# MaxChen228/pingpong-selfplay-ai

Measured on AMD Instinct MI355X. Metric: env-steps/sec (whole node) at 65536 arenas, 1/2/4/8 GPUs; CPU-ref baseline, higher is better.
Workload: dtype f64 env state / f32 QNet; 1 GPU; configs[2]: 65536 arenas/GPU, full DQN train_iterative loop (act both players + env tick + PER push/sample + double-DQN update + Adam + target sync); arenas_per_gpu=65536, global_arenas=65536, pool=8, batch=256, updates_per_vector_step=1, memory_size=1000000, parallelism=dp1 (arena shards, 1 all-reduce/update)

## Files before the change

pingpong-selfplay-ai_amd/csrc/pm_mfma.h:

```cpp
#pragma once
#include "pm_dev.h"

namespace pm {

typedef float f32x16 __attribute__((ext_vector_type(16)));
typedef __attribute__((address_space(3))) void lds_void;

constexpr int PLAIN = 4936;
enum : int {
    F_W1 = 0,
    F_W2 = 512,
    F_B1 = 4608,
    F_B2 = 4672,
    F_H = 4736,
    F_BH = 4992,
    F_SIZE = 5008,
};
static_assert(PLAIN + F_SIZE == PM_QNET_NW, "effective weight block size");

__device__ __forceinline__ int rho(int r) { return (r & 3) + 8 * (r >> 2); }

__device__ __forceinline__ float relu(float x) { return __int_as_float(max(__float_as_int(x), 0)); }

__device__ __forceinline__ void write_feature_frag_image(const float* __restrict__ p, float* __restrict__ f) {
    const int t = threadIdx.x, nt = blockDim.x;
    for (int k = t; k < 512; k += nt) {
        const int jt = k >> 8, lane = (k >> 2) & 63, s = k & 3;
        const int row = 32 * jt + (lane & 31), kk = 2 * s + (lane >> 5);
        f[F_W1 + k] = kk == 0 ? p[B1 + row] : p[W1 + row * 7 + kk - 1];
    }
    for (int k = t; k < 4096; k += nt) {
        const int e = k & 3, lane = (k >> 2) & 63, rq = (k >> 8) & 3, tt = (k >> 10) & 1, jt = k >> 11;
        const int row = 32 * jt + (lane & 31), col = 32 * tt + rho(4 * rq + e) + 4 * (lane >> 5);
        f[F_W2 + k] = p[W2 + row * 64 + col];
    }
    for (int k = t; k < 64; k += nt) {
        const int r = k & 15, h = (k >> 4) & 1, jt = k >> 5;
        f[F_B1 + k] = p[B1 + 32 * jt + rho(r) + 4 * h];
        f[F_B2 + k] = p[B2 + 32 * jt + rho(r) + 4 * h];
    }
}
__device__ __forceinline__ void write_feature_frags(const float* __restrict__ p, float* __restrict__ w) {
    for (int k = threadIdx.x; k < PM_QNET_HEAD_OFF; k += blockDim.x) w[k] = p[k];
    write_feature_frag_image(p, w + PLAIN);
}

__device__ __forceinline__ void write_head_frags(const float* heads, float* __restrict__ w) {
    const int t = threadIdx.x, nt = blockDim.x;
    for (int k = t; k < 260; k += nt) w[WH + k] = heads[k];
    float* f = w + PLAIN;
    for (int k = t; k < 256; k += nt) {
        const int c = k & 3, r = (k >> 2) & 15, tt = (k >> 6) & 1, h = k >> 7;
        f[F_H + k] = heads[c * 64 + 32 * tt + rho(r) + 4 * h];
    }
    if (t < 16) f[F_BH + t] = t < 4 ? heads[256 + t] : 0.f;
}

constexpr int kLwChunks = (F_SIZE / 4 + 63) / 64;
constexpr int kLwFloats = kLwChunks * 256;

template <int N>
__device__ __forceinline__ void copy_lds_f32(const float* __restrict__ src, float* dst) {
    const int wv = threadIdx.x >> 6, lane = threadIdx.x & 63, nw = blockDim.x >> 6;
    for (int c = wv; c * 64 < N; c += nw) {
        const int k = min(c * 64 + lane, N - 1);
        __builtin_amdgcn_global_load_lds((const void*)(src + k), (lds_void*)(dst + c * 64), 4, 0, 0);
    }
}
constexpr int pad64(int n) { return (n + 63) / 64 * 64; }
template <int N>
__device__ __forceinline__ void copy_lds_f32x4(const float* __restrict__ src, float* dst) {
    static_assert(N % 4 == 0, "whole float4s");
    const int wv = threadIdx.x >> 6, lane = threadIdx.x & 63, nw = blockDim.x >> 6;
    const float4* s4 = reinterpret_cast<const float4*>(src);
    for (int c = wv; c * 256 < N; c += nw) {
        const int k = min(c * 64 + lane, N / 4 - 1);
        __builtin_amdgcn_global_load_lds((const void*)(s4 + k), (lds_void*)(dst + c * 256), 16, 0, 0);
    }
}
constexpr int pad256(int n) { return (n + 255) / 256 * 256; }

__device__ __forceinline__ void stage_frags_lds(const float* __restrict__ w, float* lw, int rot) {
    const int wv = threadIdx.x >> 6, lane = threadIdx.x & 63, nw = blockDim.x >> 6;
    const float4* src = reinterpret_cast<const float4*>(w + PLAIN);
    float4* lw4 = reinterpret_cast<float4*>(lw);
    rot %= kLwChunks;
    for (int c0 = wv; c0 < kLwChunks; c0 += nw) {
        const int c = c0 + rot < kLwChunks ? c0 + rot : c0 + rot - kLwChunks;
// ... 140 lines not shown
__device__ __forceinline__ void tile_heads(const float* hf, const f32x16 (&c2)[2], int lane, float (&q)[3]) {
    const int h = lane >> 5;
    float v = 0.f, a0 = 0.f, a1 = 0.f, a2 = 0.f;
    const float4* hw = reinterpret_cast<const float4*>(hf + h * 128);
#pragma unroll
    for (int t = 0; t < 2; ++t) {
#pragma unroll
        for (int r = 0; r < 16; ++r) {
            const float x = relu(c2[t][r]);
            const float4 w = hw[t * 16 + r];
            v = fmaf(w.x, x, v);
            a0 = fmaf(w.y, x, a0);
            a1 = fmaf(w.z, x, a1);
            a2 = fmaf(w.w, x, a2);
        }
        __builtin_amdgcn_sched_barrier(0);
    }
    v += __shfl_xor(v, 32);
    a0 += __shfl_xor(a0, 32);
    a1 += __shfl_xor(a1, 32);
    a2 += __shfl_xor(a2, 32);
    v += hf[256];
    a0 += hf[257];
    a1 += hf[258];
    a2 += hf[259];
    const float mean = ((a0 + a1) + a2) / 3.0f;
    q[0] = v + (a0 - mean);
    q[1] = v + (a1 - mean);
    q[2] = v + (a2 - mean);
}

__device__ __forceinline__ void hidden_half(const float* lw, const float (&xs)[4], int lane, int jt, f32x16& c2) {
    const int h = lane >> 5;
    f32x16 c1[2];
    const f32x16 zero = {};
#pragma unroll
    for (int t = 0; t < 2; ++t) {
        const float4 w = reinterpret_cast<const float4*>(lw + F_W1)[t * 64 + lane];
        c1[t] = __builtin_amdgcn_mfma_f32_32x32x2f32(w.x, xs[0], zero, 0, 0, 0);
        c1[t] = __builtin_amdgcn_mfma_f32_32x32x2f32(w.y, xs[1], c1[t], 0, 0, 0);
        c1[t] = __builtin_amdgcn_mfma_f32_32x32x2f32(w.z, xs[2], c1[t], 0, 0, 0);
        c1[t] = __builtin_amdgcn_mfma_f32_32x32x2f32(w.w, xs[3], c1[t], 0, 0, 0);
    }
#pragma unroll
    for (int t = 0; t < 2; ++t)
#pragma unroll
        for (int r = 0; r < 16; ++r) c1[t][r] = relu(c1[t][r]);
    {
        const float4* b = reinterpret_cast<const float4*>(lw + F_B2 + (jt * 2 + h) * 16);
#pragma unroll
        for (int q4 = 0; q4 < 4; ++q4) {
            const float4 v = b[q4];
            c2[4 * q4 + 0] = v.x; c2[4 * q4 + 1] = v.y; c2[4 * q4 + 2] = v.z; c2[4 * q4 + 3] = v.w;
        }
    }
    const float4* w2 = reinterpret_cast<const float4*>(lw + F_W2) + lane + jt * 8 * 64;
    float4 wcur = w2[0];
#pragma unroll
    for (int g = 0; g < 8; ++g) {
        const int t = g >> 2, rq = g & 3;
        const float4 wnext = w2[((g + 1) & 7) * 64];
        c2 = __builtin_amdgcn_mfma_f32_32x32x2f32(wcur.x, c1[t][4 * rq + 0], c2, 0, 0, 0);
        c2 = __builtin_amdgcn_mfma_f32_32x32x2f32(wcur.y, c1[t][4 * rq + 1], c2, 0, 0, 0);
        c2 = __builtin_amdgcn_mfma_f32_32x32x2f32(wcur.z, c1[t][4 * rq + 2], c2, 0, 0, 0);
        c2 = __builtin_amdgcn_mfma_f32_32x32x2f32(wcur.w, c1[t][4 * rq + 3], c2, 0, 0, 0);
        wcur = wnext;
        __builtin_amdgcn_sched_barrier(0);
    }
}

__device__ __forceinline__ void heads_half(const float* hf, const f32x16& c2, int lane, int t, float (&acc)[4]) {
    const float4* hw = reinterpret_cast<const float4*>(hf + (lane >> 5) * 128) + t * 16;
#pragma unroll
    for (int r = 0; r < 16; ++r) {
        const float x = relu(c2[r]);
        const float4 w = hw[r];
        acc[0] = fmaf(w.x, x, acc[0]);
        acc[1] = fmaf(w.y, x, acc[1]);
        acc[2] = fmaf(w.z, x, acc[2]);
        acc[3] = fmaf(w.w, x, acc[3]);
    }
}

__device__ __forceinline__ void heads_finish(const float (&acc)[4], const float* hf, float (&q)[3]) {
    float v = acc[0], a0 = acc[1], a1 = acc[2], a2 = acc[3];
    v += __shfl_xor(v, 32);
    a0 += __shfl_xor(a0, 32);
    a1 += __shfl_xor(a1, 32);
    a2 += __shfl_xor(a2, 32);
    v += hf[256];
    a0 += hf[257];
    a1 += hf[258];
    a2 += hf[259];
    const float mean = ((a0 + a1) + a2) / 3.0f;
    q[0] = v + (a0 - mean);
    q[1] = v + (a1 - mean);
    q[2] = v + (a2 - mean);
}

__device__ __forceinline__ int l2_pos(int u) {
    const int t = u >> 5, v = u & 31, b = (v >> 2) & 1, r = (v & 3) + 4 * (v >> 3);
    return 2 * (16 * t + r) + b;
}
__device__ __forceinline__ int l2_unit(int q) {
    const int i = q >> 1, b = q & 1;
    return 32 * (i >> 4) + rho(i & 15) + 4 * b;
}
__device__ __forceinline__ int head_pos(int u) {
    const int t = u >> 5, v = u & 31;
    return 16 * t + (v & 3) + 4 * (v >> 3);
}

typedef float f32x4v16 __attribute__((ext_vector_type(4)));

template <int NSET>
__device__ __forceinline__ void heads_to_opw(float (&opw)[NSET][2][4][32], int set, const float* hf) {
    const int lane = threadIdx.x & 63;
#pragma unroll
    for (int it = 0; it < 4; ++it) {
        const int idx = it * 64 + lane, h = idx >> 7, j = (idx >> 5) & 3, q = idx & 31;
        opw[set][h][j][q] = hf[(h * 32 + q) * 4 + j];
    }
}

__device__ __forceinline__ float xor16_sum(float v) {
    const auto r = __builtin_amdgcn_permlane16_swap(__float_as_uint(v), __float_as_uint(v), false, false);
    return __uint_as_float(r[0]) + __uint_as_float(r[1]);
}

__device__ __forceinline__ void tile_inputs(const float* __restrict__ o, int h, float (&xs)[4]) {
    xs[0] = h ? o[0] : 1.0f;
    xs[1] = o[1 + h];
    xs[2] = o[3 + h];
    xs[3] = o[5 + h];
}

struct TilePre {
    bool have;
    float xs[4];
};

__device__ __forceinline__ void run_tiles(const float* lw, const float* __restrict__ obs, const int* list, int count,
                                          const TileOut& out, const TilePre pre) {
    const int lane = threadIdx.x & 63, wave = threadIdx.x >> 6, nw = blockDim.x >> 6;
    const int h = lane >> 5, col = lane & 31;
    const int ntiles = (count + 31) >> 5;
    int tl = wave;
    if (tl >= ntiles) return;
    int arena = list[min(tl * 32 + col, count - 1)];
    float xs[4];
    if (pre.have) {
#pragma unroll
        for (int k = 0; k < 4; ++k) xs[k] = pre.xs[k];
    } else {
        tile_inputs(obs + (size_t)arena * 7, h, xs);
    }
    for (; tl < ntiles; tl += nw) {
        const int row = tl * 32 + col;
        const bool valid = row < count;
        const int tn = tl + nw;
        int arena_n = arena;
        float xn[4] = {xs[0], xs[1], xs[2], xs[3]};
        if (tn < ntiles) {
            arena_n = list[min(tn * 32 + col, count - 1)];
            tile_inputs(obs + (size_t)arena_n * 7, h, xn);
        }
        f32x16 c2[2];
#ifdef PM_DIAG
        if (tl == wave) {
            __builtin_amdgcn_s_waitcnt(0);
            PM_BLK(5);
        }
#endif
        tile_hidden(lw, xs, lane, c2);
#ifdef PM_DIAG
        if (tl == wave) PM_BLK(6);
#endif
        float q[3];
        tile_heads(lw + F_H, c2, lane, q);
#ifdef PM_DIAG
        if (tl == wave) PM_BLK(7);
#endif
        int a = argmax3(q);
        if (out.eps >= 0.0) {
            const U4 rr = philox64((uint32_t)arena, TAG_ACT, out.ctr, out.seed);
            if (u53(rr.x, rr.y) < out.eps) a = below(rr.z, 3u);
        }
        if (h == 0 && valid) {
            if (out.act) out.act[arena] = (int8_t)a;
            if (out.q) {
                out.q[(size_t)arena * 3 + 0] = q[0];
                out.q[(size_t)arena * 3 + 1] = q[1];
                out.q[(size_t)arena * 3 + 2] = q[2];
            }
        }
        arena = arena_n;
#pragma unroll
        for (int k = 0; k < 4; ++k) xs[k] = xn[k];
    }
}

constexpr int kChunkB = 256;

struct ActGrid {
    int n, n_opp, chunk0, chunk1, side_b;
    __host__ __device__ int nb() const { return side_b ? (n + kChunkB - 1) / kChunkB : 0; }
    __host__ __device__ int na0() const { return (n + chunk0 - 1) / chunk0; }
    __host__ __device__ int na1() const { return (n + chunk1 - 1) / chunk1; }
    __host__ __device__ int blocks() const { return nb() + na0() + (n_opp - 1) * na1(); }
};

constexpr int kActBlock = 256;
constexpr int kListMax = 4096;
constexpr int kListMaxLearn = 16384;

template <int LIST>
struct ActSharedT {
    static constexpr int kList = LIST;
    float lw[kLwFloats];
    int list[LIST];
    int count;
    int wtot[16];
    int lpre[LIST / 256], loff[LIST / 256], lcnt[LIST / 256];
};
using ActShared = ActSharedT<kListMax>;
using ActSharedLearn = ActSharedT<kListMaxLearn>;
static_assert(kListMaxLearn / 256 <= 64, "one lane per list segment in act_block's scan");

template <class Sh>
__device__ __forceinline__ void act_block(Sh& sh, const ActGrid& g, const float* __restrict__ w_opp,
                                          const int32_t* __restrict__ opp, const float* __restrict__ w_B,
                                          const float* __restrict__ obsA, const float* __restrict__ obsB,
                                          TileOut outA, TileOut outB, int b,
                                          const int32_t* __restrict__ opp_list = nullptr,
                                          const int32_t* __restrict__ opp_cnt = nullptr) {
    const float* w;
    const float* obs;
    TileOut out;
    int net, lo, hi;
    bool compact;
    if (b < g.nb()) {
        w = w_B; obs = obsB; out = outB; net = -1; lo = b * kChunkB; hi = min(lo + kChunkB, g.n); compact = false;
    } else {
        b -= g.nb();
        if (b < g.na0()) { net = 0; lo = b * g.chunk0; hi = min(lo + g.chunk0, g.n); }
        else { b -= g.na0(); net = 1 + b / g.na1(); lo = (b % g.na1()) * g.chunk1; hi = min(lo + g.chunk1, g.n); }
        w = w_opp + (size_t)net * PM_QNET_NW; obs = obsA; out = outA;
        compact = opp != nullptr;
        if (!compact && net != 0) return;
    }
    __builtin_amdgcn_s_setprio(2);
    stage_frags_lds(w, sh.lw, b);
    const bool lists = compact && opp_list != nullptr && (lo & 255) == 0 && (((hi - lo) & 255) == 0 || hi == g.n);
    int ids[16];
    if (compact && !lists) compact_load(opp, lo, hi, ids);
    PM_BLK(4);
    if (lists) {
        const int g0 = lo >> 8, G = (hi - lo + 255) >> 8;
        if (threadIdx.x < 64) {
            const int lane = threadIdx.x;
            const int v = lane < G ? opp_cnt[(size_t)(g0 + lane) * g.n_opp + net] : 0;
            const int c = v & 0xFFFF;
            const int incl = wave_incl_scan_i32(c);
            if (lane < G) { sh.lpre[lane] = incl - c; sh.loff[lane] = v >> 16; sh.lcnt[lane] = c; }
            if (lane == 63) sh.count = incl;
        }
        __syncthreads();
        const int j0 = threadIdx.x & 15;
        for (int seg = threadIdx.x >> 4; seg < G; seg += blockDim.x >> 4) {
            const int c = sh.lcnt[seg], dst = sh.lpre[seg];
            const int32_t* src = opp_list + (size_t)(g0 + seg) * 256 + sh.loff[seg];
            int v[16];
#pragma unroll
            for (int r = 0; r < 16; ++r) v[r] = j0 + 16 * r < c ? src[j0 + 16 * r] : 0;
#pragma unroll
            for (int r = 0; r < 16; ++r)
                if (j0 + 16 * r < c) sh.list[dst + j0 + 16 * r] = v[r];
        }
    } else if (compact) {
        compact_scan(ids, net, lo, sh.list, &sh.count, sh.wtot);
    } else {
        if (threadIdx.x == 0) sh.count = hi - lo;
        for (int k = threadIdx.x; k < hi - lo; k += blockDim.x) sh.list[k] = lo + k;
    }
    TilePre pre{false, {0.f, 0.f, 0.f, 0.f}};
    if (!compact && !lists) {
        const int wave = threadIdx.x >> 6, lane = threadIdx.x & 63, cnt = hi - lo;
        if (wave * 32 < cnt) {
            pre.have = true;
            tile_inputs(obs + (size_t)(lo + min(wave * 32 + (lane & 31), cnt - 1)) * 7, lane >> 5, pre.xs);
        }
    }
    __syncthreads();
    PM_BLK(1);
    __builtin_amdgcn_s_setprio(0);
    run_tiles(sh.lw, obs, sh.list, sh.count, out, pre);
}

constexpr int kFeatTileFloats = 8 * 64 * 4;
__device__ __forceinline__ void store_f4_sc1(__amdgpu_buffer_rsrc_t r, int byte_off, float4 v) {
    typedef __attribute__((ext_vector_type(4))) unsigned u32x4;
    __builtin_amdgcn_raw_buffer_store_b128(*reinterpret_cast<const u32x4*>(&v), r, byte_off, 0, 16 );
}
__device__ __forceinline__ void feat_store(float* __restrict__ feat, int tl, int lane, const f32x16 (&c2)[2]) {
    const __amdgpu_buffer_rsrc_t rs = __builtin_amdgcn_make_buffer_rsrc(feat, (short)0, 0x7fffffff, 0x00020000);
    const int off = (tl * 8 * 64 + lane) * 16;
#pragma unroll
    for (int k = 0; k < 4; ++k) {
        store_f4_sc1(rs, off + k * 64 * 16, make_float4(c2[0][4 * k], c2[0][4 * k + 1], c2[0][4 * k + 2], c2[0][4 * k + 3]));
        store_f4_sc1(rs, off + (4 + k) * 64 * 16,
                     make_float4(c2[1][4 * k], c2[1][4 * k + 1], c2[1][4 * k + 2], c2[1][4 * k + 3]));
    }
}
__device__ __forceinline__ void feat_tiles(float* lw, const float* __restrict__ w, const float* __restrict__ obs, int n,
                                           int t0, int t1, float* __restrict__ feat) {
    const int wave = threadIdx.x >> 6, lane = threadIdx.x & 63, nw = blockDim.x >> 6;
    stage_frags_lds(w, lw, t0);
    int tl = t0 + wave;
    float xs[4] = {0.f, 0.f, 0.f, 0.f};
    if (tl < t1) tile_inputs(obs + (size_t)min(tl * 32 + (lane & 31), n - 1) * 7, lane >> 5, xs);
    __syncthreads();
    for (; tl < t1; tl += nw) {
        const int tn = tl + nw;
        float xn[4] = {xs[0], xs[1], xs[2], xs[3]};
        if (tn < t1) tile_inputs(obs + (size_t)min(tn * 32 + (lane & 31), n - 1) * 7, lane >> 5, xn);
        f32x16 c2[2];
        tile_hidden(lw, xs, lane, c2);
        feat_store(feat, tl, lane, c2);
#pragma unroll
        for (int k = 0; k < 4; ++k) xs[k] = xn[k];
    }
}
__device__ __forceinline__ void feat_load(const float* __restrict__ feat, int tile, int lane, f32x16 (&c2)[2]) {
    const float4* src = reinterpret_cast<const float4*>(feat) + (size_t)tile * 8 * 64 + lane;
#pragma unroll
    for (int k = 0; k < 4; ++k) {
        const float4 a = src[k * 64], b = src[(4 + k) * 64];
        c2[0][4 * k] = a.x; c2[0][4 * k + 1] = a.y; c2[0][4 * k + 2] = a.z; c2[0][4 * k + 3] = a.w;
        c2[1][4 * k] = b.x; c2[1][4 * k + 1] = b.y; c2[1][4 * k + 2] = b.z; c2[1][4 * k + 3] = b.w;
    }
}

}
```

pingpong-selfplay-ai_amd/csrc/pm_selfplay.hip:

```cpp
#include <algorithm>
#include <cmath>

#include "pm_host.h"
#include "pm_mfma.h"
#include "pm_per.h"

using namespace pm;

#ifdef PM_DIAG
static __device__ unsigned long long pm_diag_env[8][1024];
static __device__ unsigned long long pm_diag_side[4][1024];
#define PM_SIDE(k, sb, v)                                                        \
    do {                                                                         \
        if (threadIdx.x == 0 && (sb) < 1024) pm_diag_side[(k)][(sb)] = (v);      \
    } while (0)
#define PM_STAMP_MAX_NB(slot)                                                                              \
    do {                                                                                                   \
        if (threadIdx.x == 0) atomicMax(&pm_diag_buf[(slot)], (unsigned long long)__builtin_amdgcn_s_memrealtime()); \
    } while (0)
#define PM_ENV_STAMP(k, blk)                                                                   \
    do {                                                                                       \
        asm volatile("" ::: "memory");                                                         \
        if (threadIdx.x == 0 && (blk) < 1024) pm_diag_env[(k)][(blk)] = __builtin_amdgcn_s_memrealtime(); \
    } while (0)
// ... 8 lines not shown
    } while (0)
#define PM_STAMP_MAX_NB(slot) \
    do {                      \
    } while (0)
#define PM_ENV_STAMP(k, blk) \
    do {                     \
    } while (0)
#define PM_ENV_STAMP_DRAIN(k, blk) \
    do {                           \
    } while (0)
#endif

namespace {

constexpr int kBlock = 256;
static_assert(kBlock == kRowBlock, "row staging assumes kRowBlock-thread blocks");
constexpr int kLearn = 1024;
constexpr int kGradN = PM_GRAD_EPISODES;
static_assert(PM_GRAD_EPISODES == PM_QNET_NHEAD && PM_GRAD_UPDATED == kGradN + 1 && PM_GRAD_LEN >= kGradN + 2, "grad layout");
constexpr uint32_t kHashEmpty = 0xFFFFFFFFu;

__device__ __forceinline__ bool learner_active(const pm_selfplay& sp) {
    const int64_t s = sp.ctrl->size + sp.n;
    return (s < sp.cap ? s : sp.cap) >= sp.batch;
}

__device__ __forceinline__ double beta_of(const pm_selfplay& sp, int64_t frame) {
    const double b = sp.beta_start + (double)frame * (1.0 - sp.beta_start) / (double)sp.beta_frames;
    return b < 1.0 ? b : 1.0;
}

__device__ __forceinline__ float push_prio(int64_t size, float max_prio) { return size == 0 ? 1.0f : max_prio; }
__device__ __forceinline__ PushRange push_of(const pm_selfplay& sp, int64_t pos, int64_t size, float max_prio) {
    return PushRange{pos, sp.n, sp.cap, prio_pow(push_prio(size, max_prio), (float)sp.alpha)};
}
}

__device__ __forceinline__ void sample_block(const pm_selfplay& sp, int b, bool pending, PerSampleSmem& sm) {
    const pm_ctrl* c = sp.ctrl;
    const int64_t s = c->size + sp.n;
    const int64_t size = s < sp.cap ? s : sp.cap;
    const int64_t frame = c->frame_idx + 1;
    const PushRange pr = pending ? push_of(sp, c->pos, c->size, c->max_prio) : PushRange{0, 0, sp.cap, 0.f};
    const uint64_t key = sp.seed_env;
    per_sample_block(
        size >= sp.batch, size, per_tree(sp.per_work, sp.cap), pr, beta_of(sp, frame), b * PER_BS,
        min(sp.batch, b * PER_BS + PER_BS), sm,
        [&](int j) {
            const U4 r = philox64((uint32_t)j, TAG_PER, (uint64_t)frame, key);
            return u53(r.x, r.y);
        },
        [&](int j, int64_t idx, float w) {
            sp.idx[j] = idx;
            sp.isw[j] = w;
        });
}

union ActSpShared {
    ActShared act;
    PerSampleSmem per;
};
constexpr int kFeatTilesAct = 8, kFeatTilesLearn = 16;
#ifndef PM_ENV_WT
#define PM_ENV_WT 7
#endif
constexpr bool kEnvWTRows = (PM_ENV_WT & 1) != 0, kEnvWTState = (PM_ENV_WT & 2) != 0, kEnvWTObs = (PM_ENV_WT & 4) != 0;
constexpr bool kEnvWTPrio = (PM_ENV_WT & 8) != 0;
constexpr bool kEnvWTFrow = (PM_ENV_WT & 16) != 0;
__host__ __device__ inline int feat_ntiles(int n) { return (n + 31) / 32; }

__device__ __forceinline__ bool gb_current(const pm_selfplay& sp) {
    return sp.featB && sp.gB && sp.gB_ready && !sp.frow;
}
__device__ __forceinline__ uint32_t* gh_epoch(const pm_selfplay& sp) {
    return reinterpret_cast<uint32_t*>(sp.gheads + PM_GHEADS_EPOCH);
}
constexpr int kAheadPollMax = 20000;
__device__ __forceinline__ void gh_publish(const pm_selfplay& sp, int k, uint32_t tag, float v) {
    __hip_atomic_store(sp.gheads + k, ((uint64_t)tag << 32) | __float_as_uint(v), __ATOMIC_RELAXED, __HIP_MEMORY_SCOPE_AGENT);
}

struct FeatAheadSmem {
    float lw[kLwFloats];
    float hf[264];
    int ok;
};
__device__ __forceinline__ void feat_tiles_ahead(const pm_selfplay& sp, FeatAheadSmem& sm, int t0, int t1, bool force_timeout) {
    const int t = threadIdx.x, wave = t >> 6, lane = t & 63, nw = blockDim.x >> 6;
    stage_frags_lds(sp.w_B, sm.lw, t0);
    const uint32_t tag = __hip_atomic_load(gh_epoch(sp), __ATOMIC_RELAXED, __HIP_MEMORY_SCOPE_AGENT) + 1u;
    const int tl[2] = {t0 + wave, t0 + wave + nw};
    const bool has[2] = {tl[0] < t1, tl[1] < t1};
    float xs[2][4] = {{0.f, 0.f, 0.f, 0.f}, {0.f, 0.f, 0.f, 0.f}};
#pragma unroll
    for (int k = 0; k < 2; ++k)
        if (has[k]) tile_inputs(sp.obsB + (size_t)min(tl[k] * 32 + (lane & 31), sp.n - 1) * 7, lane >> 5, xs[k]);
    if (t == 0) sm.ok = 1;
    __syncthreads();
    f32x16 c2[2][2] = {};
#pragma unroll
    for (int k = 0; k < 2; ++k)
        if (has[k]) tile_hidden(sm.lw, xs[k], lane, c2[k]);
    PM_STAMP_MAX_NB(68);
    if (t < 260) {
        const int c = t & 3, r = (t >> 2) & 15, tt = (t >> 6) & 1, h = t >> 7;
        const int src = t < 256 ? c * 64 + 32 * tt + rho(r) + 4 * h : t;
        uint64_t g = 0;
        bool got = false;
        for (int it = 0; !force_timeout && it < kAheadPollMax; ++it) {
            g = __hip_atomic_load(sp.gheads + src, __ATOMIC_RELAXED, __HIP_MEMORY_SCOPE_AGENT);
            if ((uint32_t)(g >> 32) == tag) { got = true; break; }
            __builtin_amdgcn_s_sleep(2);
        }
        if (got) sm.hf[t] = __uint_as_float((uint32_t)g);
        else sm.ok = 0;
    }
    __syncthreads();
    PM_STAMP_MAX_NB(69);
    const bool ok = sm.ok != 0;
#pragma unroll
    for (int k = 0; k < 2; ++k) {
        if (!has[k]) continue;
        const int arena = tl[k] * 32 + (lane & 31);
        int a = PM_GB_NONE;
        if (ok) {
            float q[3];
            tile_heads(sm.hf, c2[k], lane, q);
            a = argmax3(q);
        } else {
            feat_store(sp.featB, tl[k], lane, c2[k]);
        }
        if (lane < 32 && arena < sp.n) sp.gB[arena] = (int8_t)a;
    }
}

__global__ __launch_bounds__(kActBlock, 4) void k_act_sp(const pm_selfplay sp, int part) {
    __shared__ __attribute__((aligned(16))) ActSpShared sh;
    PM_BLK(0);
    const int nsb = part == PM_ACT_A ? 0 : (sp.batch + PER_BS - 1) / PER_BS;
    {
        const ActGrid g{sp.n, sp.n_pool + 1, sp.chunk_A, sp.chunk_P, part == PM_ACT_A ? 0 : 1};
        const int fb = (int)blockIdx.x - nsb - g.blocks();
        if (fb >= 0) {
            const int t0 = fb * kFeatTilesAct;
            feat_tiles(sh.act.lw, sp.w_B, sp.obsB, sp.n, t0, min(t0 + kFeatTilesAct, feat_ntiles(sp.n)), sp.featB);
            return;
        }
    }
    if ((int)blockIdx.x < nsb) {
        PM_STAMP(64);
        sample_block(sp, (int)blockIdx.x, true, sh.per);
        PM_STAMP(65);
        PM_BLK_END();
        return;
    }
    if ((int)blockIdx.x == nsb) PM_STAMP_ANY(70);
    const ActGrid g{sp.n, sp.n_pool + 1, sp.chunk_A, sp.chunk_P, part == PM_ACT_A ? 0 : 1};
    const TileOut outA{sp.aA, nullptr, -1.0, 0, 0};
    const TileOut outB{sp.aB, nullptr, -1.0, 0, 0};
    act_block(sh.act, g, sp.w_opp, sp.n_pool > 0 ? sp.opp : nullptr, sp.w_B, sp.obsA, sp.obsB, outA, outB,
              (int)blockIdx.x - nsb, sp.n_pool + 1 <= kListNets ? sp.opp_list : nullptr, sp.opp_cnt);
    PM_BLK_END();
}

__device__ __forceinline__ void batch_row_fwd(const pm_selfplay& sp, const float* lw, const float* hf0, const float* hf1,
                                              int64_t id, bool nxt, int lane, f32x16 (&c2)[2], float (&qb)[3],
                                              float (&qt)[3], float (&rb)[2]) {
    float xs[4];
    const float* tr = sp.trans + id * PM_TRANS_F;
    tile_inputs(tr + (nxt ? 8 : 0), lane >> 5, xs);
    rb[0] = tr[7];
    rb[1] = tr[15];
    tile_hidden(lw, xs, lane, c2);
    tile_heads(hf0, c2, lane, qb);
    tile_heads(hf1, c2, lane, qt);
}

template <bool WT = false>
__device__ __forceinline__ void store_hfeat(float* hfeat, int j, bool nxt, int lane, const f32x16 (&c2)[2],
                                            const float (&qb)[3], const float (&qt)[3], const float (&rb)[2]) {
    float* row = hfeat + (size_t)j * 80;
    const int h = lane >> 5;
    if (!nxt) {
#pragma unroll
        for (int t = 0; t < 2; ++t)
#pragma unroll
            for (int q = 0; q < 16; ++q) st_out<WT>(&row[32 * t + rho(q) + 4 * h], relu(c2[t][q]));
    }
    if (h == 0) {
        if (!nxt) {
            st_out<WT>(&row[64], qb[0]); st_out<WT>(&row[65], qb[1]); st_out<WT>(&row[66], qb[2]);
            st_out<WT>(&row[67], rb[0]);
            st_out<WT>(&row[71], rb[1]);
        } else {
            st_out<WT>(&row[68], qb[0]); st_out<WT>(&row[69], qb[1]); st_out<WT>(&row[70], qb[2]);
            st_out<WT>(&row[72], qt[0]); st_out<WT>(&row[73], qt[1]); st_out<WT>(&row[74], qt[2]);
        }
    }
}

__device__ __forceinline__ void env_fwd_block(const pm_selfplay& sp, int f, bool pending = true) {
    __shared__ __attribute__((aligned(16))) float lw[kLwFloats];
    __shared__ __attribute__((aligned(16))) float hf[2][264];
    if (!learner_active(sp)) return;
    stage_frags_lds(sp.w_B, lw, f * 5);
    for (int k = threadIdx.x; k < 2 * 264; k += blockDim.x) hf[k / 264][k % 264] = sp.learn_heads[k];
    __syncthreads();
    const int lane = threadIdx.x & 63, B = sp.batch;
    const int r0 = f * 128 + (int)(threadIdx.x >> 6) * 32;
    if (r0 >= 2 * B) return;
    const int r = min(r0 + (lane & 31), 2 * B - 1);
    const bool nxt = r >= B;
    const int j = nxt ? r - B : r;
    const int64_t id = sp.idx[j];
    const pm_ctrl* c = sp.ctrl;
// ... 409 lines not shown
__device__ __forceinline__ void adam_consts(const pm_selfplay& sp, int64_t ts, ApplySmem& sm) {
    const double bc1 = 1.0 - pow(sp.beta1, (double)ts);
    const double bc2 = 1.0 - pow(sp.beta2, (double)ts);
    sm.ak[0] = (float)(sp.lr / bc1);
    sm.ak[1] = (float)sqrt(bc2);
}
__device__ __forceinline__ void adam_const_lane(const pm_selfplay& sp, int64_t ts, ApplySmem& sm, int which) {
    const double bc = 1.0 - pow(which ? sp.beta2 : sp.beta1, (double)ts);
    sm.ak[which] = which ? (float)sqrt(bc) : (float)(sp.lr / bc);
}

__device__ __forceinline__ void load_apply_inputs(const pm_selfplay& sp, ApplySmem& sm, bool with_grad) {
    copy_lds_f32x4<PM_QNET_NHEAD>(sp.paramsB + PM_QNET_HEAD_OFF, sm.hp);
    copy_lds_f32x4<PM_QNET_NHEAD>(sp.paramsT + PM_QNET_HEAD_OFF, sm.tmu);
    copy_lds_f32x4<PM_QNET_NHEAD>(sp.adam_m, sm.m);
    copy_lds_f32x4<PM_QNET_NHEAD>(sp.adam_v, sm.v);
    if (with_grad)
        for (int k = threadIdx.x; k < PM_QNET_NHEAD + 2; k += blockDim.x) sm.g[k] = sp.grad[k];
}

__device__ __forceinline__ void derive_weights(const pm_selfplay& sp, ApplySmem& sm, bool gh_on = false, uint32_t gh_tag = 0) {
    const int t = threadIdx.x;
    float* lh = sp.learn_heads;
    const int g = (t - 256) >> 8, u = (t - 256) & 255;
    if (t >= 256 && g == 0) {
        fold_heads_from(sm.hp, nullptr, sm.nact, PM_FOLD_TRAIN_FRESH, sm.heads[0], sp.paramsB + PM_QNET_EPS_OFF, u, 256);
        if (gh_on) {
            gh_publish(sp, u, gh_tag, sm.heads[0][u]);
            if (u < 4) gh_publish(sp, 256 + u, gh_tag, sm.heads[0][256 + u]);
            PM_STAMP_T(22, 256);
        }
    } else if (t >= 256 && g == 1) {
        fold_heads_from(sm.hp, nullptr, sm.ntrain, PM_FOLD_TRAIN_FRESH, sm.heads[1], lh + 528, u, 256);
    } else if (t >= 256 && g == 2) {
        fold_heads_from(sm.tmu, nullptr, nullptr, PM_FOLD_EVAL, sm.heads[2], nullptr, u, 256);
    }
    __syncthreads();
    write_head_frags(sm.heads[0], sp.w_B);
    heads_to_frags(sm.heads[1], lh);
    heads_to_frags(sm.heads[2], lh + 264);
}

__device__ __forceinline__ void derive_weights_lds(ApplySmem& sm) {
    const int t = threadIdx.x;
    const int g = (t - 256) >> 8, u = (t - 256) & 255;
    if (t >= 256 && g == 1) {
        fold_heads_from(sm.hp, nullptr, sm.ntrain, PM_FOLD_TRAIN_FRESH, sm.heads[1], nullptr, u, 256);
    } else if (t >= 256 && g == 2) {
        fold_heads_from(sm.tmu, nullptr, nullptr, PM_FOLD_EVAL, sm.heads[2], nullptr, u, 256);
    }
    __syncthreads();
}

__device__ __forceinline__ void gen_both_noises(const pm_selfplay& sp, ApplySmem& sm, uint64_t act_ctr,
                                                uint64_t train_ctr) {
    const int t = threadIdx.x, half = blockDim.x / 2;
    if (t < half) gen_noise(sp.seed_net, TAG_NOISE_ACT, act_ctr, sm.nact, t, half);
    else gen_noise(sp.seed_net, TAG_NOISE_TRAIN, train_ctr, sm.ntrain, t - half, half);
}
__device__ __forceinline__ void gen_both_noises_on(const pm_selfplay& sp, ApplySmem& sm, uint64_t act_ctr,
                                                   uint64_t train_ctr, int t0) {
    const int u = (int)threadIdx.x - t0;
    if (u < 0 || u >= 512) return;
    if (u < 256) gen_noise(sp.seed_net, TAG_NOISE_ACT, act_ctr, sm.nact, u, 256);
    else gen_noise(sp.seed_net, TAG_NOISE_TRAIN, train_ctr, sm.ntrain, u - 256, 256);
}

__device__ __forceinline__ void adam_one(const pm_selfplay& sp, ApplySmem& sm, int k, float gsum, bool store = true) {
    const float step_size = sm.ak[0], bc2s = sm.ak[1];
    const float g = gsum / (float)sp.world;
    float m = sm.m[k], v = sm.v[k], p = sm.hp[k];
    m = m + (float)(1.0 - sp.beta1) * (g - m);
    v = v * (float)sp.beta2 + (float)(1.0 - sp.beta2) * g * g;
    const float denom = sqrtf(v) / bc2s + (float)sp.adam_eps;
    p = p - step_size * (m / denom);
    if (store) {
        sp.paramsB[PM_QNET_HEAD_OFF + k] = p;
        sp.adam_m[k] = m;
        sp.adam_v[k] = v;
    }
    sm.hp[k] = p;
    sm.m[k] = m;
    sm.v[k] = v;
}
__device__ __forceinline__ void apply_adam(const pm_selfplay& sp, ApplySmem& sm) {
    const int t = threadIdx.x, nt = blockDim.x;
    if (sm.g[kGradN + 1] > 0.5f)
        for (int k = t; k < PM_QNET_NHEAD; k += nt) adam_one(sp, sm, k, sm.g[k]);
}
__device__ __forceinline__ void apply_finish(const pm_selfplay& sp, ApplySmem& sm, const pm_ctrl& cs, int mode,
                                             bool gh_on = false, uint32_t gh_tag = 0) {
    const int t = threadIdx.x, nt = blockDim.x;
    const bool train = sm.g[kGradN + 1] > 0.5f;
    const int64_t ts = cs.train_steps + (train ? 1 : 0);
    const uint64_t step = cs.step;
    PM_STAMP(20);
    if (train && ts % sp.target_update_interval == 0) {
        for (int k = t; k < PM_QNET_NHEAD; k += nt) sm.tmu[k] = sm.hp[k];
        for (int k = t; k < PM_QNET_NP; k += nt) {
            const int h = k - PM_QNET_HEAD_OFF;
            sp.paramsT[k] = (h >= 0 && h < PM_QNET_NHEAD) ? sm.hp[h] : sp.paramsB[k];
        }
        __syncthreads();
    }
    derive_weights(sp, sm, gh_on, gh_tag);
    PM_STAMP(21);
    if (t == 0) {
        pm_ctrl* c = sp.ctrl;
        if (mode & PM_UPD_FIRST) {
            const double e = sm.eps_next;
            c->epsilon = e > sp.min_epsilon ? e : sp.min_epsilon;
        }
        if (train) { c->train_steps = ts; c->frame_idx = cs.frame_idx + 1; }
        if (mode & PM_UPD_LAST) {
            c->pos = (cs.pos + sp.n) % sp.cap;
            const int64_t s = cs.size + sp.n;
            c->size = s < sp.cap ? s : sp.cap;
            c->step = step + 1;
        }
    }
}

template <typename Emit>
__device__ __forceinline__ void push_rows_fwd(const pm_selfplay& sp, const float* lw, const float* hf,
                                              const int64_t* sidx, const int* plist, const int* pcnt, int wv, int lane,
                                              Emit emit) {
    int pre[5] = {0, 0, 0, 0, 0};
#pragma unroll
    for (int w = 0; w < 4; ++w) pre[w + 1] = pre[w] + pcnt[w];
    const int np = pre[4];
    if (wv * 32 >= 2 * np) return;
    const int rr = min(wv * 32 + (lane & 31), 2 * np - 1);
    const bool nxt = rr >= np;
    const int k = nxt ? rr - np : rr;
    const int w = k >= pre[3] ? 3 : k >= pre[2] ? 2 : k >= pre[1] ? 1 : 0;
    const int pw = k >= pre[3] ? pre[3] : k >= pre[2] ? pre[2] : k >= pre[1] ? pre[1] : 0;
    const int j = plist[w * 64 + k - pw];
    f32x16 c2[2];
    float qb[3], qt[3], rb[2];
    batch_row_fwd(sp, lw, hf, hf + 264, sidx[j], nxt, lane, c2, qb, qt, rb);
    if (wv * 32 + (lane & 31) < 2 * np) emit(j, nxt, lane, c2, qb, qt, rb);
}

constexpr int kPushPollMax = 20000;
constexpr int PM_CTRL_PUSH_TIMEOUT = 1;
constexpr int PM_CTRL_NAN_PRIO = 2;
__device__ __forceinline__ bool push_handoff(int mode, bool train) { return (mode & PM_UPD_FIRST) && train; }
__device__ __forceinline__ int* push_flag(const pm_selfplay& sp) {
    return reinterpret_cast<int*>(sp.hfeat + (size_t)2 * sp.batch * 80);
}
__device__ __forceinline__ int push_token(const pm_ctrl& cs) { return (int)((uint32_t)cs.step + 1u); }
__device__ __forceinline__ uint32_t* tr_epoch(const pm_selfplay& sp) {
    return reinterpret_cast<uint32_t*>(sp.hfeat + (size_t)2 * sp.batch * 80) + 1;
}
constexpr int kPushGF = 76;
constexpr int kPushGN = 75;
__device__ __forceinline__ uint64_t* push_granules(const pm_selfplay& sp) {
    return reinterpret_cast<uint64_t*>(sp.hfeat + (size_t)(2 * sp.batch + 8) * 80);
}
__device__ __forceinline__ void push_publish(uint64_t* g, uint32_t tag, float v) {
    __hip_atomic_store(g, ((uint64_t)tag << 32) | __float_as_uint(v), __ATOMIC_RELAXED, __HIP_MEMORY_SCOPE_AGENT);
}

__device__ __forceinline__ bool push_wait(const pm_selfplay& sp, const pm_ctrl& cs) {
    const int* flag = push_flag(sp);
    const int tok = push_token(cs);
// ... 638 lines not shown
            const double base = which < 0 ? sp.epsilon_decay : which ? sp.beta2 : sp.beta1;
            const double ex = which < 0 ? (double)(float)s : (double)(cs.train_steps + 1);
            const double p = pow(base, ex);
            if (which < 0) {
                if (first) sm.ap.eps_next = cs.epsilon * p;
            } else {
                const double bc = 1.0 - p;
                sm.ap.ak[which] = which ? (float)sqrt(bc) : (float)(sp.lr / bc);
            }
        }
        gen_both_noises_on(sp, sm.ap, cs.step + 1, (uint64_t)(cs.train_steps + (train0 ? 1 : 0)) + 1, kLearn / 2);
    }
    {
        const float s = wave_sum(lossp), mp = wave_max(prio);
#pragma unroll
        for (int k = 0; k < 4; ++k) cf[k] = wave_sum(cf[k]);
        if (lane == 0) {
            sm.red[wv][1] = s; sm.red[wv][2] = mp;
#pragma unroll
            for (int k = 0; k < 4; ++k) sm.red[wv][3 + k] = cf[k];
        }
    }
    asm volatile("s_waitcnt vmcnt(0)" ::: "memory");
    __syncthreads();
    PM_STAMP(3);

    float mpx = 0.f;
    if (train) {
        mpx = sm.red[0][2];
        for (int w = 1; w < 16; ++w) mpx = fmaxf(mpx, sm.red[w][2]);
    }
    const float leaf_v = act ? prio_pow(prio, (float)sp.alpha) : 0.f;
    if (tr) {
        if (t < B) tr_publish(sp, t, __float_as_uint(leaf_v), tr_tag);
        if (t == B) tr_publish(sp, B, __float_as_uint(train ? fmaxf(cs.max_prio, mpx) : cs.max_prio), tr_tag);
        if (t == B + 1) tr_publish(sp, B + 1, train ? 1u : 0u, tr_tag);
    }
    if (train) {
        if (act && sm.hwin[slot] == t) {
            sp.prios[id] = prio;
            tree.leaf[id] = leaf_v;
            if (prio != prio) atomicOr(&sp.ctrl->status, PM_CTRL_NAN_PRIO);
        }
        if (t == 0) {
            float l = 0.f;
            for (int w = 0; w < 16; ++w) l += sm.red[w][1];
            sm.loss_out = l / (float)B;
        }
        const int col = t & 63;
        float g[4] = {0.f, 0.f, 0.f, 0.f};
        const int j0 = wv * 16, j1 = min(j0 + 16, B);
        for (int j = j0; j < j1; ++j) {
            const float4 k4 = *reinterpret_cast<const float4*>(sm.coef[j]);
            const float h = sm.Hs[j][col];
            g[0] = fmaf(k4.x, h, g[0]);
            g[1] = fmaf(k4.y, h, g[1]);
            g[2] = fmaf(k4.z, h, g[2]);
            g[3] = fmaf(k4.w, h, g[3]);
        }
#pragma unroll
        for (int r = 0; r < 4; ++r) sm.u.gpart[wv][r * 64 + col] = g[r];
    }
    const float max_prio_next = train ? fmaxf(cs.max_prio, mpx) : cs.max_prio;
    if (!tr) __threadfence_block();
    __syncthreads();
    PM_STAMP(4);

    const PushRange next = last ? push_of(sp, (cs.pos + sp.n) % sp.cap, s_after, max_prio_next)
                                : PushRange{0, 0, sp.cap, 0.f};
    if (train) {
        if (t < 256) {
            float g = 0.f;
#pragma unroll
            for (int w = 0; w < 16; ++w) g += sm.u.gpart[w][t];
            const int row = t >> 6, col = t & 63;
            float* gs = sm.ap.g;
            const int a = row - 1;
            const int kmu = row == 0 ? col : 130 + a * 64 + col, ksg = row == 0 ? 65 + col : 325 + a * 64 + col;
            const float gsg = g * sm.eps_tr[row == 0 ? P_VWEP - PM_QNET_EPS_OFF + col
                                                     : P_AWEP - PM_QNET_EPS_OFF + a * 64 + col];
            gs[kmu] = g;
            gs[ksg] = gsg;
            if (sp.fuse_apply) {
                adam_one(sp, sm.ap, kmu, g);
                adam_one(sp, sm.ap, ksg, gsg);
            }
        } else if (t < 260) {
            const int k = t - 256;
            float g = 0.f;
            for (int w = 0; w < 16; ++w) g += sm.red[w][3 + k];
            float* gs = sm.ap.g;
            const int kmu = k == 0 ? 64 : 322 + k - 1, ksg = k == 0 ? 129 : 517 + k - 1;
            const float gsg = g * sm.eps_tr[k == 0 ? P_VBEP - PM_QNET_EPS_OFF : P_ABEP - PM_QNET_EPS_OFF + k - 1];
            gs[kmu] = g;
            gs[ksg] = gsg;
            if (sp.fuse_apply) {
                adam_one(sp, sm.ap, kmu, g);
                adam_one(sp, sm.ap, ksg, gsg);
            }
        }
        if ((ahead & 1) && t < 260) {
            fold_heads_from(sm.ap.hp, nullptr, sm.ap.nact, PM_FOLD_TRAIN_FRESH, sm.ap.heads[0], nullptr, t, kLearn);
            gh_publish(sp, t, gh_tag, sm.ap.heads[0][t]);
            PM_STAMP(22);
        }
        PM_STAMP(8); PM_STAMP_T(9, 960);
        if (!tr) {
            const int j = min(t >> 2, B - 1);
            const int64_t sb = sm.sidx[j] / PER_SUB;
            const double v = per_sub_sum4(tree.leaf, sb, next);
            if ((t & 3) == 0) tree.sub[sb] = v;
        }
        PM_STAMP(10); PM_STAMP_T(11, 960);
    } else {
        for (int k = t; k < kGradN; k += kLearn) sm.ap.g[k] = 0.f;
    }
    if (t == 0) { sm.ap.g[kGradN] = (float)ep_fin; sm.ap.g[kGradN + 1] = train ? 1.f : 0.f; }
    if (!tr) {
        const RingNodes rn = ring_nodes(next, PER_SUB);
        const double csub = per_sub_pushed_sum(next);
        for (int64_t k = t; k < rn.count(); k += kLearn) {
            const int64_t sb = rn.at(k);
            if (per_sub_pushed(sb, next)) tree.sub[sb] = csub;
        }
        PM_STAMP(12); PM_STAMP_T(13, 960);
        if (wv == 0) {
            const int g = lane >> 2;
            const bool ok = g < 4 && (g < 2 ? rn.na : rn.nb) > 0;
            const int64_t sb = !ok ? 0 : g == 0 ? rn.a0 : g == 1 ? rn.a0 + rn.na - 1 : g == 2 ? 0 : rn.nb - 1;
            const double v = per_sub_sum4(tree.leaf, sb, next);
            if (ok && (lane & 3) == 0 && !per_sub_pushed(sb, next)) tree.sub[sb] = v;
        }
    }
    PM_STAMP(14); PM_STAMP_T(15, 960);
    if (!tr) __threadfence_block();
    __syncthreads();
    PM_STAMP(5);
    for (int k = t; k < kGradN + 2; k += kLearn) sp.grad[k] = sm.ap.g[k];
    if (!tr && act && sm.hwin[slot] == t) {
        const int64_t ch = id / PER_CHUNK;
        tree.chunk[ch] = per_chunk_sum(tree, ch);
    }
    if (!tr) {
        const RingNodes rn = ring_nodes(next, PER_CHUNK);
        for (int64_t k = t; k < rn.count(); k += kLearn) {
            const int64_t ch = rn.at(k);
            tree.chunk[ch] = per_chunk_sum(tree, ch);
        }
    }
    PM_STAMP(6);
    if (sp.fuse_apply && first && !waited) {
        if (t == 0) push_wait(sp, cs);
        __syncthreads();
    }
    if (sp.fuse_apply) apply_finish(sp, sm.ap, cs, mode, (ahead & 1) && !train, gh_tag);
    if (t == 0) {
        if (ahead & 1) __hip_atomic_store(gh_epoch(sp), gh_tag, __ATOMIC_RELAXED, __HIP_MEMORY_SCOPE_AGENT);
        if (first) {
            c->ep_step = ep_fin;
            c->episodes = cs.episodes + ep_fin;
            c->ep_A = cs.ep_A + sm.ctot[1]; c->win_A = cs.win_A + sm.ctot[2];
            c->ep_P = cs.ep_P + sm.ctot[3]; c->win_P = cs.win_P + sm.ctot[4];
            c->reward_B = cs.reward_B + (double)sm.ctot[5];
        }
        if (train) {
            c->last_loss = sm.loss_out;
            c->max_prio = max_prio_next;
        }
    }
    PM_STAMP(7);
}

__global__ __launch_bounds__(kLearn) void k_adam(const pm_selfplay sp, int mode) {
    __shared__ ApplySmem sm;
    const int t = threadIdx.x;
    const pm_ctrl cs = *sp.ctrl;
    load_apply_inputs(sp, sm, true);
    const float D = sp.grad[kGradN], upd = sp.grad[kGradN + 1];
    const int64_t ts = cs.train_steps + (upd > 0.5f ? 1 : 0);
    gen_both_noises_on(sp, sm, cs.step + 1, (uint64_t)ts + 1, kLearn / 2);
    if (t >= kLearn - 2) adam_const_lane(sp, cs.train_steps + 1, sm, t - (kLearn - 2));
// ... 928 lines not shown
```

Measured before the change: 2.328 billion env-steps/s.

## Compute Q-net dueling heads with 4x4x1 MFMA from staged LDS weight layout

Replaces the scalar FMA dueling-head computation in the act and feature-ahead paths with chains of mfma_f32_4x4x1f32 over a padded LDS weight layout (opw), staged alongside the fragment weights. The ahead path processes two tiles together with interleaved MFMAs. Adam updates for the paired mu/sigma gradients are merged into one interleaved helper to expose ILP. It adds LDS footprint and a layout-translation step, and relies on the MFMA lane mapping matching the c2 fragment layout.

```diff
diff --git a/pingpong-selfplay-ai_amd/csrc/pm_mfma.h b/pingpong-selfplay-ai_amd/csrc/pm_mfma.h
--- a/pingpong-selfplay-ai_amd/csrc/pm_mfma.h
+++ b/pingpong-selfplay-ai_amd/csrc/pm_mfma.h
@@ -4,6 +4,7 @@
 namespace pm {
 
 typedef float f32x16 __attribute__((ext_vector_type(16)));
+typedef float f32x4v16 __attribute__((ext_vector_type(4)));
 typedef __attribute__((address_space(3))) void lds_void;
 
 constexpr int PLAIN = 4936;
@@ -310,21 +311,79 @@
     }
 }
 
-__device__ __forceinline__ void heads_finish(const float (&acc)[4], const float* hf, float (&q)[3]) {
+__device__ __forceinline__ void heads_finish_b(const float (&acc)[4], const float* bh, float (&q)[3]) {
     float v = acc[0], a0 = acc[1], a1 = acc[2], a2 = acc[3];
     v += __shfl_xor(v, 32);
     a0 += __shfl_xor(a0, 32);
     a1 += __shfl_xor(a1, 32);
     a2 += __shfl_xor(a2, 32);
-    v += hf[256];
-    a0 += hf[257];
-    a1 += hf[258];
-    a2 += hf[259];
+    v += bh[0];
+    a0 += bh[1];
+    a1 += bh[2];
+    a2 += bh[3];
     const float mean = ((a0 + a1) + a2) / 3.0f;
     q[0] = v + (a0 - mean);
     q[1] = v + (a1 - mean);
     q[2] = v + (a2 - mean);
 }
+__device__ __forceinline__ void heads_finish(const float (&acc)[4], const float* hf, float (&q)[3]) {
+    heads_finish_b(acc, hf + 256, q);
+}
+
+constexpr int kOpwStride = 36;
+constexpr int kOpwFloats = 8 * kOpwStride;
+__device__ __forceinline__ int opw_slot(int k) { return (4 * (k >> 7) + (k & 3)) * kOpwStride + ((k >> 2) & 31); }
+
+__device__ __forceinline__ const float4* opw_row(const float* opw, int lane) {
+    return reinterpret_cast<const float4*>(opw + (4 * (lane >> 5) + (lane & 3)) * kOpwStride);
+}
+
+__device__ __forceinline__ void heads_half_mfma(const float* opw, const f32x16& c2, int lane, int t, f32x4v16& acc) {
+    const float4* aw = opw_row(opw, lane) + 4 * t;
+    float4 w = aw[0];
+#pragma unroll
+    for (int k = 0; k < 4; ++k) {
+        const float4 wn = aw[(k + 1) & 3];
+        acc = __builtin_amdgcn_mfma_f32_4x4x1f32(w.x, relu(c2[4 * k + 0]), acc, 0, 0, 0);
+        acc = __builtin_amdgcn_mfma_f32_4x4x1f32(w.y, relu(c2[4 * k + 1]), acc, 0, 0, 0);
+        acc = __builtin_amdgcn_mfma_f32_4x4x1f32(w.z, relu(c2[4 * k + 2]), acc, 0, 0, 0);
+        acc = __builtin_amdgcn_mfma_f32_4x4x1f32(w.w, relu(c2[4 * k + 3]), acc, 0, 0, 0);
+        w = wn;
+    }
+}
+__device__ __forceinline__ void heads_finish_mfma(const f32x4v16& acc, const float* bh, float (&q)[3]) {
+    const float a[4] = {acc[0], acc[1], acc[2], acc[3]};
+    heads_finish_b(a, bh, q);
+}
+__device__ __forceinline__ void tile_heads_mfma(const float* opw, const float* bh, const f32x16 (&c2)[2], int lane,
+                                                float (&q)[3]) {
+    f32x4v16 acc = {0.f, 0.f, 0.f, 0.f};
+    heads_half_mfma(opw, c2[0], lane, 0, acc);
+    heads_half_mfma(opw, c2[1], lane, 1, acc);
+    heads_finish_mfma(acc, bh, q);
+}
+__device__ __forceinline__ void tile_heads_mfma2(const float* opw, const float* bh, const f32x16 (&ca)[2],
+                                                 const f32x16 (&cb)[2], int lane, float (&qa)[3], float (&qb)[3]) {
+    const float4* aw = opw_row(opw, lane);
+    f32x4v16 xa = {0.f, 0.f, 0.f, 0.f}, xb = {0.f, 0.f, 0.f, 0.f};
+    float4 w = aw[0];
+#pragma unroll
+    for (int k = 0; k < 8; ++k) {
+        const float4 wn = aw[(k + 1) & 7];
+        const int t = k >> 2, r = 4 * (k & 3);
+        xa = __builtin_amdgcn_mfma_f32_4x4x1f32(w.x, relu(ca[t][r + 0]), xa, 0, 0, 0);
+        xb = __builtin_amdgcn_mfma_f32_4x4x1f32(w.x, relu(cb[t][r + 0]), xb, 0, 0, 0);
+        xa = __builtin_amdgcn_mfma_f32_4x4x1f32(w.y, relu(ca[t][r + 1]), xa, 0, 0, 0);
+        xb = __builtin_amdgcn_mfma_f32_4x4x1f32(w.y, relu(cb[t][r + 1]), xb, 0, 0, 0);
+        xa = __builtin_amdgcn_mfma_f32_4x4x1f32(w.z, relu(ca[t][r + 2]), xa, 0, 0, 0);
+        xb = __builtin_amdgcn_mfma_f32_4x4x1f32(w.z, relu(cb[t][r + 2]), xb, 0, 0, 0);
+        xa = __builtin_amdgcn_mfma_f32_4x4x1f32(w.w, relu(ca[t][r + 3]), xa, 0, 0, 0);
+        xb = __builtin_amdgcn_mfma_f32_4x4x1f32(w.w, relu(cb[t][r + 3]), xb, 0, 0, 0);
+        w = wn;
+    }
+    heads_finish_mfma(xa, bh, qa);
+    heads_finish_mfma(xb, bh, qb);
+}
 
 __device__ __forceinline__ int l2_pos(int u) {
     const int t = u >> 5, v = u & 31, b = (v >> 2) & 1, r = (v & 3) + 4 * (v >> 3);
@@ -338,8 +397,6 @@
     const int t = u >> 5, v = u & 31;
     return 16 * t + (v & 3) + 4 * (v >> 3);
 }
-
-typedef float f32x4v16 __attribute__((ext_vector_type(4)));
 
 template <int NSET>
 __device__ __forceinline__ void heads_to_opw(float (&opw)[NSET][2][4][32], int set, const float* hf) {
@@ -368,8 +425,8 @@
     float xs[4];
 };
 
-__device__ __forceinline__ void run_tiles(const float* lw, const float* __restrict__ obs, const int* list, int count,
-                                          const TileOut& out, const TilePre pre) {
+__device__ __forceinline__ void run_tiles(const float* lw, const float* opw, const float* __restrict__ obs,
+                                          const int* list, int count, const TileOut& out, const TilePre pre) {
     const int lane = threadIdx.x & 63, wave = threadIdx.x >> 6, nw = blockDim.x >> 6;
     const int h = lane >> 5, col = lane & 31;
     const int ntiles = (count + 31) >> 5;
@@ -405,7 +462,7 @@
         if (tl == wave) PM_BLK(6);
 #endif
         float q[3];
-        tile_heads(lw + F_H, c2, lane, q);
+        tile_heads_mfma(opw, lw + F_BH, c2, lane, q);
 #ifdef PM_DIAG
         if (tl == wave) PM_BLK(7);
 #endif
@@ -446,6 +503,7 @@
 struct ActSharedT {
     static constexpr int kList = LIST;
     float lw[kLwFloats];
+    float opw[kOpwFloats];
     int list[LIST];
     int count;
     int wtot[16];
@@ -479,6 +537,7 @@
     }
     __builtin_amdgcn_s_setprio(2);
     stage_frags_lds(w, sh.lw, b);
+    const float hv = threadIdx.x < 256 ? w[PLAIN + F_H + threadIdx.x] : 0.f;
     const bool lists = compact && opp_list != nullptr && (lo & 255) == 0 && (((hi - lo) & 255) == 0 || hi == g.n);
     int ids[16];
     if (compact && !lists) compact_load(opp, lo, hi, ids);
@@ -519,10 +578,11 @@
             tile_inputs(obs + (size_t)(lo + min(wave * 32 + (lane & 31), cnt - 1)) * 7, lane >> 5, pre.xs);
         }
     }
+    if (threadIdx.x < 256) sh.opw[opw_slot(threadIdx.x)] = hv;
     __syncthreads();
     PM_BLK(1);
     __builtin_amdgcn_s_setprio(0);
-    run_tiles(sh.lw, obs, sh.list, sh.count, out, pre);
+    run_tiles(sh.lw, sh.opw, obs, sh.list, sh.count, out, pre);
 }
 
 constexpr int kFeatTileFloats = 8 * 64 * 4;
diff --git a/pingpong-selfplay-ai_amd/csrc/pm_selfplay.hip b/pingpong-selfplay-ai_amd/csrc/pm_selfplay.hip
--- a/pingpong-selfplay-ai_amd/csrc/pm_selfplay.hip
+++ b/pingpong-selfplay-ai_amd/csrc/pm_selfplay.hip
@@ -114,7 +114,7 @@
 
 struct FeatAheadSmem {
     float lw[kLwFloats];
-    float hf[264];
+    __attribute__((aligned(16))) float hf[kOpwFloats + 8];
     int ok;
 };
 __device__ __forceinline__ void feat_tiles_ahead(const pm_selfplay& sp, FeatAheadSmem& sm, int t0, int t1, bool force_timeout) {
@@ -144,25 +144,30 @@
             if ((uint32_t)(g >> 32) == tag) { got = true; break; }
             __builtin_amdgcn_s_sleep(2);
         }
-        if (got) sm.hf[t] = __uint_as_float((uint32_t)g);
+        if (got) sm.hf[t < 256 ? opw_slot(t) : kOpwFloats + t - 256] = __uint_as_float((uint32_t)g);
         else sm.ok = 0;
     }
     __syncthreads();
     PM_STAMP_MAX_NB(69);
     const bool ok = sm.ok != 0;
+    int a[2] = {PM_GB_NONE, PM_GB_NONE};
+    if (ok) {
+        float q0[3], q1[3];
+        if (has[1]) {
+            tile_heads_mfma2(sm.hf, sm.hf + kOpwFloats, c2[0], c2[1], lane, q0, q1);
+            a[0] = argmax3(q0);
+            a[1] = argmax3(q1);
+        } else if (has[0]) {
+            tile_heads_mfma(sm.hf, sm.hf + kOpwFloats, c2[0], lane, q0);
+            a[0] = argmax3(q0);
+        }
+    }
 #pragma unroll
     for (int k = 0; k < 2; ++k) {
         if (!has[k]) continue;
         const int arena = tl[k] * 32 + (lane & 31);
-        int a = PM_GB_NONE;
-        if (ok) {
-            float q[3];
-            tile_heads(sm.hf, c2[k], lane, q);
-            a = argmax3(q);
-        } else {
-            feat_store(sp.featB, tl[k], lane, c2[k]);
-        }
-        if (lane < 32 && arena < sp.n) sp.gB[arena] = (int8_t)a;
+        if (!ok) feat_store(sp.featB, tl[k], lane, c2[k]);
+        if (lane < 32 && arena < sp.n) sp.gB[arena] = (int8_t)a[k];
     }
 }
 
@@ -738,6 +743,32 @@
     sm.hp[k] = p;
     sm.m[k] = m;
     sm.v[k] = v;
+}
+__device__ __forceinline__ void adam_two(const pm_selfplay& sp, ApplySmem& sm, int k0, float g0s, int k1, float g1s) {
+    const float step_size = sm.ak[0], bc2s = sm.ak[1];
+    const float g0 = g0s / (float)sp.world, g1 = g1s / (float)sp.world;
+    float m0 = sm.m[k0], v0 = sm.v[k0], p0 = sm.hp[k0];
+    float m1 = sm.m[k1], v1 = sm.v[k1], p1 = sm.hp[k1];
+    m0 = m0 + (float)(1.0 - sp.beta1) * (g0 - m0);
+    m1 = m1 + (float)(1.0 - sp.beta1) * (g1 - m1);
+    v0 = v0 * (float)sp.beta2 + (float)(1.0 - sp.beta2) * g0 * g0;
+    v1 = v1 * (float)sp.beta2 + (float)(1.0 - sp.beta2) * g1 * g1;
+    const float d0 = sqrtf(v0) / bc2s + (float)sp.adam_eps;
+    const float d1 = sqrtf(v1) / bc2s + (float)sp.adam_eps;
+    p0 = p0 - step_size * (m0 / d0);
+    p1 = p1 - step_size * (m1 / d1);
+    sm.hp[k0] = p0;
+    sm.hp[k1] = p1;
+    sp.paramsB[PM_QNET_HEAD_OFF + k0] = p0;
+    sp.adam_m[k0] = m0;
+    sp.adam_v[k0] = v0;
+    sp.paramsB[PM_QNET_HEAD_OFF + k1] = p1;
+    sp.adam_m[k1] = m1;
+    sp.adam_v[k1] = v1;
+    sm.m[k0] = m0;
+    sm.v[k0] = v0;
+    sm.m[k1] = m1;
+    sm.v[k1] = v1;
 }
 __device__ __forceinline__ void apply_adam(const pm_selfplay& sp, ApplySmem& sm) {
     const int t = threadIdx.x, nt = blockDim.x;
@@ -1542,8 +1573,7 @@
             gs[kmu] = g;
             gs[ksg] = gsg;
             if (sp.fuse_apply) {
-                adam_one(sp, sm.ap, kmu, g);
-                adam_one(sp, sm.ap, ksg, gsg);
+                adam_two(sp, sm.ap, kmu, g, ksg, gsg);
             }
         } else if (t < 260) {
             const int k = t - 256;
@@ -1555,8 +1585,7 @@
             gs[kmu] = g;
             gs[ksg] = gsg;
             if (sp.fuse_apply) {
-                adam_one(sp, sm.ap, kmu, g);
-                adam_one(sp, sm.ap, ksg, gsg);
+                adam_two(sp, sm.ap, kmu, g, ksg, gsg);
             }
         }
         if ((ahead & 1) && t < 260) {
```

Result: faster. 2.357 billion env-steps/s (median of 6 runs) (+1.2%).
